# NazirNayal8/RbA

Hardware: AMD Instinct MI355X
Metric: images/sec @1024x2048 Swin-B-1dl (RbA inference hot path) (higher is better)
Workload: dtype f32 (f16x3 split-MFMA GEMMs, fp32 accumulate)

## Files before the change

### include/rba_hip.h

```cpp
#ifndef RBA_HIP_H
#define RBA_HIP_H

#include <stdint.h>

#ifdef __cplusplus
extern "C" {
#endif

int rba_hip_version(void);

int rba_set_concurrent_streams(int n);

int rba_reduce_f32(const float* mask, const float* cls_prob, float* rba, float* sem_seg, int32_t* argmax,
                   int Q, int K, int64_t HW, int score_mode, void* stream);

int rba_reduce_ws_f32(const float* mask, const float* cls_prob, float* rba, float* sem_seg, int32_t* argmax, int Q, int K,
                      int64_t HW, int score_mode, void* workspace, void* stream);

int rba_reduce_up4_f32(const float* mask_lowres, const float* cls_prob, float* rba, float* sem_seg,
                       int32_t* argmax, int Q, int K, int h, int w, int crop_h, int crop_w, int score_mode, void* stream);

int rba_resample_bilinear_f32(const float* in, const float* add, float* out, int C, int h, int w, int H, int W,
                              void* stream);

int rba_ms_deform_attn_fwd_f32(const float* value, const int64_t* spatial_shapes, const int64_t* level_start_index,
                               const float* sampling_loc, const float* attn_weight, float* out,
                               int N, int S, int M, int D, int L, int Lq, int P, void* stream);
int rba_ms_deform_attn_fwd_f64(const double* value, const int64_t* spatial_shapes, const int64_t* level_start_index,
                               const double* sampling_loc, const double* attn_weight, double* out,
                               int N, int S, int M, int D, int L, int Lq, int P, void* stream);

int rba_ms_deform_attn_bwd_f32(const float* value, const int64_t* spatial_shapes, const int64_t* level_start_index,
                               const float* sampling_loc, const float* attn_weight, const float* grad_out,
                               float* grad_value, float* grad_sampling_loc, float* grad_attn_weight,
                               int N, int S, int M, int D, int L, int Lq, int P, void* stream);
int rba_ms_deform_attn_bwd_f64(const double* value, const int64_t* spatial_shapes, const int64_t* level_start_index,
                               const double* sampling_loc, const double* attn_weight, const double* grad_out,
                               double* grad_value, double* grad_sampling_loc, double* grad_attn_weight,
                               int N, int S, int M, int D, int L, int Lq, int P, void* stream);

int rba_msda_prepare_f32(const float* raw, const float* reference_points, const int64_t* spatial_shapes, float* loc, float* attw,
                         int64_t rows, int M, int L, int P, void* stream);

int rba_msda_fused_f32(const float* value, const int64_t* spatial_shapes, const int64_t* level_start_index, const float* raw,
                       const float* reference_points, float* out, int N, int S, int M, int D, int L, int Lq, int P, void* stream);

int64_t rba_masked_xattn_workspace_bytes(int B, int Q, int S, int nH);
int rba_masked_xattn_f32(const float* q, const float* k, const float* v, const float* mask_logits, float* out,
                         float* workspace, int B, int Q, int S, int nH, int hd, void* stream);

int rba_mask_logits_f32(const float* embed, const float* feat, float* out, int B, int Q, int C, int64_t N,
                        void* stream);
int rba_mask_logits_f16x3_f32(const float* embed, const float* feat, float* out, int B, int Q, int C, int64_t N,
                              void* stream);

int rba_swin_window_attn_f32(const float* qkv, const float* qkv_bias, const float* bias, const float* bias_frag,
                             float* out, int B, int H, int W, int nH, int hd, int ws, int shift, void* stream);
int64_t rba_swin_bias_fragments_elems(int nH, int ws);
int rba_swin_bias_fragments_f32(const float* bias, float* frag, int nH, int ws, void* stream);

int64_t rba_group_norm_workspace_bytes(int B, int C, int HW, int G);
int rba_group_norm_f32(const float* x, const float* gamma, const float* beta, float* y, float* workspace,
                       int B, int C, int HW, int G, float eps, int relu, void* stream);

int64_t rba_group_norm_nhwc_workspace_bytes(int B, int P, int C, int G);
int rba_group_norm_nhwc_f32(const float* x, const float* gamma, const float* beta, float* y, float* workspace, int B, int P, int C,
                            int G, float eps, int relu, void* stream);
int rba_resample_bilinear_nhwc_f32(const float* in, const float* add, float* out, int C, int h, int w, int H, int W, void* stream);

int rba_add_layer_norm_f32(const float* x, const float* t, const float* t_bias, const float* gamma, const float* beta,
                           float* sum_out, float* y, int64_t rows, int C, float eps, void* stream);

int rba_merge_layer_norm_f32(const float* x, const float* gamma, const float* beta, float* y, int B, int H, int W, int Cin, float eps,
                             void* stream);

int rba_skinny_linear_f32(const float* x, const float* weight, const float* bias, float* out, int M, int N, int K,
                          int relu, void* stream);
int rba_skinny_linear_add_f32(const float* x, const float* x_add, int add_cols, const float* weight, const float* bias, float* out,
                              int M, int N, int K, int relu, int seg_n, void* stream);

int rba_split_weight_bf16x3(const float* weight, void* packed, int N, int K, void* stream);
int rba_split_linear_f32(const float* x, const void* weight_packed, const float* bias, float* out, int64_t M, int N, int K,
                         int act, void* stream);

int rba_split_weight_f16x2(const float* weight, void* packed, int N, int K, void* stream);
int rba_split_linear_f16x3_f32(const float* x, const void* weight_packed, const float* bias, float* out, int64_t M, int N, int K,
                               int act, void* stream);
int rba_split_linear_f16x3_res_f32(const float* x, const void* weight_packed, const float* bias, const float* residual, float* out,
                                   int64_t M, int N, int K, void* stream);

int rba_add_layer_norm_frag_f32(const float* x, const float* t, const float* t_bias, const float* gamma, const float* beta,
                                float* sum_out, void* y_frag, int64_t rows, int C, float eps, void* stream);
int rba_split_linear_f16x3_frag_f32(const void* x_frag, const void* weight_packed, const float* bias, const float* residual, float* out,
                                    int64_t M, int N, int K, int act, void* stream);
int rba_swin_window_attn_split_out_f32(const float* qkv, const float* qkv_bias, const float* bias_frag, void* out_frag, int B, int H, int W,
                                       int nH, int hd, int ws, int shift, void* stream);
int rba_swin_attn_block_supported(int C, int ws);
int64_t rba_swin_attn_block_weight_bytes(int C);
int rba_swin_attn_block_pack_f32(const float* qkv_weight, const float* proj_weight, void* image, int C, void* stream);
int rba_swin_attn_block_f32(float* x, float* y2, const float* norm1_weight, const float* norm1_bias, float eps1, const void* weight_image,
                            const float* qkv_bias, const float* bias_frag, const float* proj_bias, const float* norm2_weight,
                            const float* norm2_bias, float eps2, int B, int H, int W, int C, int ws, int shift, void* stream);
int rba_swin_attn_qkv_supported(int C, int ws);
int rba_swin_attn_qkv_split_out_f32(const float* x, void* out_frag, const float* norm1_weight, const float* norm1_bias, float eps1,
                                    const void* weight_image, const float* qkv_bias, const float* bias_frag, int B, int H, int W, int C, int ws,
                                    int shift, void* stream);
int rba_resample_bilinear_nhwc_split_out_f32(const float* in, const float* add, void* out_frag, int C, int h, int w, int H, int W,
                                             int64_t row0, void* stream);

int rba_resample_bilinear_nhwc_gn_f32(const float* in, const float* in_mr, const float* in_gamma, const float* in_beta, int in_relu,
                                      const float* add, const float* add_mr, const float* add_gamma, const float* add_beta, void* out,
                                      int split_out, int C, int G, int h, int w, int H, int W, int64_t row0, void* stream);
int rba_group_norm_nhwc_stats_f32(const float* x, float* mr, float* workspace, int B, int P, int C, int G, float eps, void* stream);
int rba_conv3x3_nhwc_f16x3_split_in_f32(const void* x_frag, const void* weight_packed, const float* bias, float* out, int B, int H, int W,
                                        int C, int N, void* stream);
int rba_swin_mlp_fused_f16x3_f32(const float* x, const void* w1_packed, const float* b1, const void* w2_packed, const float* b2,
                                 const float* residual, float* out, int64_t M, int C, int HID, void* stream);
int rba_swin_mlp_fused_ln_f16x3_f32(float* x, const float* norm_weight, const float* norm_bias, float eps, const void* w1_packed, const float* b1,
                                    const void* w2_packed, const float* b2, int64_t M, int C, int HID, void* stream);
int rba_split_linear_f16x3_gelu_split_out(const void* x, int x_is_split, const void* weight_packed, const float* bias, void* out_frag,
                                          int64_t M, int N, int K, void* stream);

int rba_split_linear_nchw_out_f32(const float* x, const void* weight_packed, const float* bias, float* out, int64_t M, int N,
                                  int K, int rows_per_image, void* stream);

int rba_split_linear_nchw_out_f16x3_f32(const float* x, const void* weight_packed, const float* bias, float* out, int64_t M, int N, int K,
                                        int rows_per_image, void* stream);

int rba_split_linear_nchw_out_gn_f16x3_f32(const float* x, const float* mr, const float* gamma, const float* beta, int G, int relu,
                                           const void* weight_packed, const float* bias, float* out, int64_t M, int N, int K,
                                           int rows_per_image, void* stream);

int rba_conv3x3_nhwc_f32(const float* x, const void* weight_packed, const float* bias, float* out, int B, int H, int W, int C,
                         int N, void* stream);

int rba_conv3x3_nhwc_f16x3_f32(const float* x, const void* weight_packed, const float* bias, float* out, int B, int H, int W, int C,
                               int N, void* stream);

int rba_split_linear_f16x3_gn_moments_f32(const float* x, const void* weight_packed, const float* bias, float* out, int64_t M, int N, int K,
                                          int rows_per_image, int G, float* moments, void* stream);
int rba_conv3x3_nhwc_f16x3_split_in_gn_moments_f32(const void* x_frag, const void* weight_packed, const float* bias, float* out, int B, int H,
                                                   int W, int C, int N, int G, float* moments, void* stream);
int rba_group_norm_nhwc_merge_f32(const float* moments, float* mr, int B, int G, int splits, float eps, void* stream);

int rba_patch_im2col_u8(const uint8_t* image, float* out, int h, int w, int Hp, int Wp, const float* mean, const float* std, void* stream);
int rba_patch_im2col_f32(const float* image, float* out, int h, int w, int Hp, int Wp, const float* mean, const float* std, void* stream);

int rba_gaussian_blur_f32(const float* in, float* out, int H, int W, int kernel_size, float sigma, void* stream);

int rba_quad_mean_f32(const float* v, float* out, int64_t rows, int S, void* stream);
int rba_softmax_drop_last_f32(const float* logits, float* prob, int64_t rows, int K1, void* stream);

int rba_threshold_u8(const float* score, uint8_t* out, int64_t n, float threshold, void* stream);
int rba_morph3x3_u8(const uint8_t* in, uint8_t* out, int H, int W, int dilate, void* stream);
int rba_ccl4_roots_i32(const uint8_t* mask, int32_t* roots, int H, int W, void* stream);

int rba_bn_relu_conv1x1_f32(const float* x, const float* scale, const float* shift, const float* weight, const float* bias, float* out,
// ... 23 lines not shown
```

### rba_amd/_lib.py

```python
import ctypes
import os

_HERE = os.path.dirname(os.path.abspath(__file__))
LIB_PATH = os.environ.get("RBA_HIP_LIB") or os.path.join(_HERE, "csrc", "librba_hip.so")
KNOBS_LIB_PATH = os.path.join(_HERE, "csrc", "librba_hip_knobs.so")

_c_f32p = ctypes.c_void_p
_i = ctypes.c_int
_i64 = ctypes.c_int64
_vp = ctypes.c_void_p

SIGNATURES = {
    "rba_hip_version": [],
    "rba_set_concurrent_streams": [_i],
    "rba_reduce_f32": [_vp, _vp, _vp, _vp, _vp, _i, _i, _i64, _i, _vp],
    "rba_reduce_ws_f32": [_vp, _vp, _vp, _vp, _vp, _i, _i, _i64, _i, _vp, _vp],
    "rba_reduce_up4_f32": [_vp, _vp, _vp, _vp, _vp, _i, _i, _i, _i, _i, _i, _i, _vp],
    "rba_resample_bilinear_f32": [_vp, _vp, _vp, _i, _i, _i, _i, _i, _vp],
    "rba_ms_deform_attn_fwd_f32": [_vp, _vp, _vp, _vp, _vp, _vp, _i, _i, _i, _i, _i, _i, _i, _vp],
    "rba_ms_deform_attn_fwd_f64": [_vp, _vp, _vp, _vp, _vp, _vp, _i, _i, _i, _i, _i, _i, _i, _vp],
    "rba_ms_deform_attn_bwd_f32": [_vp, _vp, _vp, _vp, _vp, _vp, _vp, _vp, _vp, _i, _i, _i, _i, _i, _i, _i, _vp],
    "rba_ms_deform_attn_bwd_f64": [_vp, _vp, _vp, _vp, _vp, _vp, _vp, _vp, _vp, _i, _i, _i, _i, _i, _i, _i, _vp],
    "rba_msda_prepare_f32": [_vp, _vp, _vp, _vp, _vp, _i64, _i, _i, _i, _vp],
    "rba_resample_bilinear_nhwc_gn_f32": [_vp, _vp, _vp, _vp, _i, _vp, _vp, _vp, _vp, _vp, _i, _i, _i, _i, _i, _i, _i, _i64, _vp],
    "rba_group_norm_nhwc_stats_f32": [_vp, _vp, _vp, _i, _i, _i, _i, ctypes.c_float, _vp],
    "rba_msda_fused_f32": [_vp, _vp, _vp, _vp, _vp, _vp, _i, _i, _i, _i, _i, _i, _i, _vp],
    "rba_masked_xattn_workspace_bytes": [_i, _i, _i, _i],
    "rba_masked_xattn_f32": [_vp, _vp, _vp, _vp, _vp, _vp, _i, _i, _i, _i, _i, _vp],
    "rba_mask_logits_f32": [_vp, _vp, _vp, _i, _i, _i, _i64, _vp],
    "rba_mask_logits_f16x3_f32": [_vp, _vp, _vp, _i, _i, _i, _i64, _vp],
    "rba_swin_window_attn_f32": [_vp, _vp, _vp, _vp, _vp, _i, _i, _i, _i, _i, _i, _i, _vp],
    "rba_swin_window_attn_split_out_f32": [_vp, _vp, _vp, _vp, _i, _i, _i, _i, _i, _i, _i, _vp],
    "rba_swin_bias_fragments_elems": [_i, _i],
    "rba_swin_attn_block_supported": [_i, _i],
    "rba_swin_attn_block_weight_bytes": [_i],
    "rba_swin_attn_qkv_supported": [_i, _i],
    "rba_swin_attn_qkv_split_out_f32": [_vp, _vp, _vp, _vp, ctypes.c_float, _vp, _vp, _vp, _i, _i, _i, _i, _i, _i, _vp],
    "rba_swin_attn_block_pack_f32": [_vp, _vp, _vp, _i, _vp],
    "rba_swin_attn_block_f32": [_vp, _vp, _vp, _vp, ctypes.c_float, _vp, _vp, _vp, _vp, _vp, _vp, ctypes.c_float, _i, _i, _i, _i, _i, _i, _vp],
    "rba_swin_bias_fragments_f32": [_vp, _vp, _i, _i, _vp],
    "rba_skinny_linear_f32": [_vp, _vp, _vp, _vp, _i, _i, _i, _i, _vp],
    "rba_skinny_linear_add_f32": [_vp, _vp, _i, _vp, _vp, _vp, _i, _i, _i, _i, _i, _vp],
    "rba_split_weight_bf16x3": [_vp, _vp, _i, _i, _vp],
    "rba_split_linear_f32": [_vp, _vp, _vp, _vp, _i64, _i, _i, _i, _vp],
    "rba_split_weight_f16x2": [_vp, _vp, _i, _i, _vp],
    "rba_split_linear_f16x3_f32": [_vp, _vp, _vp, _vp, _i64, _i, _i, _i, _vp],
    "rba_split_linear_f16x3_res_f32": [_vp, _vp, _vp, _vp, _vp, _i64, _i, _i, _vp],
    "rba_split_linear_f16x3_frag_f32": [_vp, _vp, _vp, _vp, _vp, _i64, _i, _i, _i, _vp],
    "rba_swin_mlp_fused_f16x3_f32": [_vp, _vp, _vp, _vp, _vp, _vp, _vp, _i64, _i, _i, _vp],
    "rba_swin_mlp_fused_ln_f16x3_f32": [_vp, _vp, _vp, ctypes.c_float, _vp, _vp, _vp, _vp, _i64, _i, _i, _vp],
    "rba_split_linear_f16x3_gelu_split_out": [_vp, _i, _vp, _vp, _vp, _i64, _i, _i, _vp],
    "rba_split_linear_nchw_out_f32": [_vp, _vp, _vp, _vp, _i64, _i, _i, _i, _vp],
    "rba_split_linear_nchw_out_f16x3_f32": [_vp, _vp, _vp, _vp, _i64, _i, _i, _i, _vp],
    "rba_split_linear_f16x3_gn_moments_f32": [_vp, _vp, _vp, _vp, _i64, _i, _i, _i, _i, _vp, _vp],
    "rba_conv3x3_nhwc_f16x3_split_in_gn_moments_f32": [_vp, _vp, _vp, _vp, _i, _i, _i, _i, _i, _i, _vp, _vp],
    "rba_group_norm_nhwc_merge_f32": [_vp, _vp, _i, _i, _i, ctypes.c_float, _vp],
    "rba_split_linear_nchw_out_gn_f16x3_f32": [_vp, _vp, _vp, _vp, _i, _i, _vp, _vp, _vp, _i64, _i, _i, _i, _vp],
    "rba_conv3x3_nhwc_f32": [_vp, _vp, _vp, _vp, _i, _i, _i, _i, _i, _vp],
    "rba_conv3x3_nhwc_f16x3_f32": [_vp, _vp, _vp, _vp, _i, _i, _i, _i, _i, _vp],
    "rba_conv3x3_nhwc_f16x3_split_in_f32": [_vp, _vp, _vp, _vp, _i, _i, _i, _i, _i, _vp],
    "rba_resample_bilinear_nhwc_split_out_f32": [_vp, _vp, _vp, _i, _i, _i, _i, _i, _i64, _vp],
    "rba_patch_im2col_u8": [_vp, _vp, _i, _i, _i, _i, _vp, _vp, _vp],
    "rba_patch_im2col_f32": [_vp, _vp, _i, _i, _i, _i, _vp, _vp, _vp],
    "rba_group_norm_nhwc_workspace_bytes": [_i, _i, _i, _i],
    "rba_group_norm_nhwc_f32": [_vp, _vp, _vp, _vp, _vp, _i, _i, _i, _i, ctypes.c_float, _i, _vp],
    "rba_resample_bilinear_nhwc_f32": [_vp, _vp, _vp, _i, _i, _i, _i, _i, _vp],
    "rba_bn_relu_conv1x1_f32": [_vp, _vp, _vp, _vp, _vp, _vp, _i, _i, _i, _i64, _vp],
    "rba_resample_bilinear_ac_f32": [_vp, _vp, _i, _i, _i, _i, _i, _vp],
    "rba_gaussian_blur_f32": [_vp, _vp, _i, _i, _i, ctypes.c_float, _vp],
    "rba_quad_mean_f32": [_vp, _vp, _i64, _i, _vp],
    "rba_softmax_drop_last_f32": [_vp, _vp, _i64, _i, _vp],
    "rba_threshold_u8": [_vp, _vp, _i64, ctypes.c_float, _vp],
    "rba_morph3x3_u8": [_vp, _vp, _i, _i, _i, _vp],
    "rba_ccl4_roots_i32": [_vp, _vp, _i, _i, _vp],
    "rba_add_layer_norm_f32": [_vp, _vp, _vp, _vp, _vp, _vp, _vp, _i64, _i, ctypes.c_float, _vp],
    "rba_add_layer_norm_frag_f32": [_vp, _vp, _vp, _vp, _vp, _vp, _vp, _i64, _i, ctypes.c_float, _vp],
    "rba_merge_layer_norm_f32": [_vp, _vp, _vp, _vp, _i, _i, _i, _i, ctypes.c_float, _vp],
    "rba_group_norm_workspace_bytes": [_i, _i, _i, _i],
    "rba_group_norm_f32": [_vp, _vp, _vp, _vp, _vp, _i, _i, _i, _i, ctypes.c_float, _i, _vp],
    "rba_token_linear_pack_f16x2": [_vp, _vp, _i, _i, _vp],
    "rba_token_linear_f32": [_vp, _vp, _vp, _vp, _vp, _vp, _vp, ctypes.c_float, _vp, _i64, _i, _i, _i, _vp],
    "rba_token_linear_multi_f32": [_vp, _vp, _i, _i64, _i, _vp],
}

class TokenLinearProblem(ctypes.Structure):
    _fields_ = [("x_add", ctypes.c_void_p), ("packed", ctypes.c_void_p), ("bias", ctypes.c_void_p), ("out", ctypes.c_void_p),
                ("N", ctypes.c_int), ("ld_out", ctypes.c_int), ("act", ctypes.c_int)]


EXPECTED_ABI = 191

_lib = None


class RbaHipError(RuntimeError):
    pass


def load():
    global _lib
    if _lib is not None:
        return _lib
    _lib = _open(LIB_PATH)
    return _lib


_handles = {}


def _open(path):
    if path in _handles:
        return _handles[path]
    import torch
    if not os.path.exists(path):
        raise RbaHipError(
            f"{path} not found: build it with `python -m rba_amd.csrc.build` (hipcc --offload-arch=gfx950; --knobs for the knobs build). "
            "rba_amd has no CPU or PyTorch fallback for its HIP kernels.")
    lib = ctypes.CDLL(path)
    for name, argtypes in SIGNATURES.items():
        try:
            fn = getattr(lib, name)
        except AttributeError as e:
            raise RbaHipError(f"{path} does not export {name}; rebuild it") from e
        fn.argtypes = argtypes
        fn.restype = ctypes.c_int64 if name.endswith(("_bytes", "_elems")) else ctypes.c_int
    abi = int(lib.rba_hip_version())
    if abi != EXPECTED_ABI:
        raise RbaHipError(f"{path} has ABI version {abi}, these bindings are written for {EXPECTED_ABI}; rebuild it "
                          "(python -m rba_amd.csrc.build)")
    _handles[path] = lib
    return lib


class use_library:

    def __init__(self, path):
        self.path = path

    def __enter__(self):
        global _lib
        self.prev = _lib
        _lib = _open(self.path)
        return _lib

    def __exit__(self, *exc):
        global _lib
        _lib = self.prev
        return False


def knob(name):
    try:
        return ctypes.c_int.in_dll(load(), name)
    except ValueError as e:
        raise RbaHipError(f"{name} is a compile-time constant in the product library: run on the knobs build (RBA_HIP_LIB={KNOBS_LIB_PATH} or "
                          "rba_amd._lib.use_library(KNOBS_LIB_PATH); python -m rba_amd.csrc.build --knobs)") from e


def hip_error_string(code: int) -> str:
    try:
# ... 12 lines not shown
```

### rba_amd/csrc/layer_norm.hip

```cpp
#include "common.h"
#include "../../include/rba_hip.h"

namespace {

struct MergeGeom {
  int H, W, Cin;
};

template <int G, int NV, bool MERGE = false, bool FRAG = false, int WAVES = 4>
__global__ __launch_bounds__(64 * WAVES) void add_layer_norm_kernel(const float* x, const float* __restrict__ t,
                                                             const float* __restrict__ tb, const float* __restrict__ gamma,
                                                             const float* __restrict__ beta, float* sum_out ,
                                                             float* __restrict__ y, int64_t rows, int C, float eps,
                                                             MergeGeom mg = MergeGeom{0, 0, 0}) {
  constexpr int RPW = 64 / G;
  const int lane = threadIdx.x & 63, sub = lane % G, rsel = lane / G;
  const int64_t row = ((int64_t)blockIdx.x * WAVES + (threadIdx.x >> 6)) * RPW + rsel;
  constexpr bool TR = FRAG && WAVES == 8 && G == 64;
  __shared__ __attribute__((aligned(16))) rba_u32x4 tr_lds[TR ? NV * 64 * 8 : 1];
  const bool rvalid = row < rows;
  const int64_t base = (rvalid ? row : 0) * C;
  const int nv4 = C >> 2;
  int mi = 0, mj = 0;
  int64_t mb = 0;
// ... 49 lines not shown
    }
  }
#pragma unroll
  for (int o = G / 2; o > 0; o >>= 1) sq += __shfl_xor(sq, o, RBA_WAVE);
  const float rstd = 1.0f / sqrtf(sq / (float)C + eps);
  if (!TR && !rvalid) return;
#pragma unroll
  for (int j = 0; j < NV; ++j) {
    const int c4 = sub + j * G;
    if (c4 < nv4) {
      if (sum_out && rvalid) *reinterpret_cast<f32x4*>(sum_out + base + 4 * c4) = v[j];
      const f32x4 gj = EARLY ? g4[EARLY ? j : 0] : *reinterpret_cast<const f32x4*>(gamma + 4 * c4);
      const f32x4 bj = EARLY ? b4[EARLY ? j : 0] : *reinterpret_cast<const f32x4*>(beta + 4 * c4);
      const f32x4 o = (v[j] - mean) * rstd * gj + bj;
      if (FRAG) {
        uint32_t h[2], l[2];
        rba_split_f16x2(o.x, o.y, h[0], l[0]);
        rba_split_f16x2(o.z, o.w, h[1], l[1]);
        const bool odd = c4 & 1;
        const uint32_t s0 = odd ? h[0] : l[0], s1 = odd ? h[1] : l[1];
        const uint32_t r0 = __builtin_amdgcn_mov_dpp(s0, 0xB1, 0xf, 0xf, true), r1 = __builtin_amdgcn_mov_dpp(s1, 0xB1, 0xf, 0xf, true);
        const rba_u32x4 piece = odd ? (rba_u32x4){r0, r1, l[0], l[1]} : (rba_u32x4){h[0], h[1], r0, r1};
        const int k8 = c4 >> 1;
        if (TR) {
          const int pcol = (((k8 >> 2) * 4 + (k8 & 1) * 2 + (odd ? 1 : 0)) << 1) + ((k8 >> 1) & 1);
          const int r8 = threadIdx.x >> 6;
          tr_lds[pcol * 8 + (r8 ^ (pcol & 7))] = piece;
        } else {
          const int64_t off = ((row >> 5) * (int64_t)(C >> 5) + (k8 >> 2)) * 4096 + ((k8 & 1) * 2 + (odd ? 1 : 0)) * 1024 +
                              (((k8 >> 1) & 1) * 32 + (int)(row & 31)) * 16;
          *reinterpret_cast<rba_u32x4*>(reinterpret_cast<char*>(y) + off) = piece;
        }
      } else {
        *reinterpret_cast<f32x4*>(y + base + 4 * c4) = o;
      }
    }
  }
  if (TR) {
    __syncthreads();
    const int64_t row0 = (int64_t)blockIdx.x * 8;
    char* img = reinterpret_cast<char*>(y) + ((row0 >> 5) * (int64_t)(C >> 5)) * 4096 + (int)(row0 & 31) * 16;
    const int npc = nv4;
    for (int u = threadIdx.x; u < npc * 8; u += 64 * WAVES) {
      const int pcol = u >> 3, r8 = u & 7;
      const int x = pcol >> 1;
      if (row0 + r8 < rows)
        *reinterpret_cast<rba_u32x4*>(img + (int64_t)(x >> 2) * 4096 + (x & 3) * 1024 + (pcol & 1) * 512 + r8 * 16) = tr_lds[pcol * 8 + (r8 ^ (pcol & 7))];
    }
  }
}

template <int G, int NV, bool FRAG = false>
int launch(const float* x, const float* t, const float* tb, const float* gamma, const float* beta, float* sum_out, float* y,
           int64_t rows, int C, float eps, hipStream_t st) {
  const int64_t rpb = 4 * (64 / G);
  const int64_t blocks = (rows + rpb - 1) / rpb;
  if (blocks > 0x7fffffffLL) return (int)hipErrorInvalidValue;
  hipLaunchKernelGGL((add_layer_norm_kernel<G, NV, false, FRAG>), dim3((unsigned)blocks), dim3(256), 0, st, x, t, tb, gamma, beta, sum_out, y,
                     rows, C, eps);
  return rba_launch_status();
}

template <int NV>
int launch_frag8(const float* x, const float* t, const float* tb, const float* gamma, const float* beta, float* sum_out, float* y,
                 int64_t rows, int C, float eps, hipStream_t st) {
  const int64_t blocks = (rows + 7) / 8;
  if (blocks > 0x7fffffffLL) return (int)hipErrorInvalidValue;
  hipLaunchKernelGGL((add_layer_norm_kernel<64, NV, false, true, 8>), dim3((unsigned)blocks), dim3(512), 0, st, x, t, tb, gamma, beta, sum_out,
                     y, rows, C, eps);
  return rba_launch_status();
}

template <int G, int NV>
int launch_merge(const float* x, const float* gamma, const float* beta, float* y, int64_t rows, int C, float eps, MergeGeom mg,
                 hipStream_t st) {
  const int64_t rpb = 4 * (64 / G);
  const int64_t blocks = (rows + rpb - 1) / rpb;
  if (blocks > 0x7fffffffLL) return (int)hipErrorInvalidValue;
  hipLaunchKernelGGL((add_layer_norm_kernel<G, NV, true>), dim3((unsigned)blocks), dim3(256), 0, st, x, nullptr, nullptr, gamma, beta, nullptr,
                     y, rows, C, eps, mg);
  return rba_launch_status();
}

}

extern "C" int rba_merge_layer_norm_f32(const float* x, const float* gamma, const float* beta, float* y, int B, int H, int W, int Cin,
                                        float eps, void* stream) {
  RBA_CHECK_ARG(B >= 0 && H >= 1 && W >= 1 && Cin >= 4 && Cin % 4 == 0 && 4 * Cin <= 8192);
  if (B == 0) return 0;
  RBA_CHECK_ARG(x && gamma && beta && y);
  RBA_CHECK_ARG((((uintptr_t)x | (uintptr_t)gamma | (uintptr_t)beta | (uintptr_t)y) & 15) == 0);
  rba_begin();
  hipStream_t st = (hipStream_t)stream;
  const int C = 4 * Cin, nv4 = C / 4;
  const int64_t rows = (int64_t)B * ((H + 1) / 2) * ((W + 1) / 2);
  const MergeGeom mg{H, W, Cin};
#define RBA_L(G, NV) return launch_merge<G, NV>(x, gamma, beta, y, rows, C, eps, mg, st)
  if (nv4 <= 16) RBA_L(16, 1);
  if (nv4 <= 32) RBA_L(32, 1);
  if (nv4 <= 64) RBA_L(64, 1);
  if (nv4 <= 128) RBA_L(64, 2);
  if (nv4 <= 256) RBA_L(64, 4);
  if (nv4 <= 512) RBA_L(64, 8);
  if (nv4 <= 1024) RBA_L(64, 16);
  RBA_L(64, 32);
#undef RBA_L
}

extern "C" int rba_add_layer_norm_f32(const float* x, const float* t, const float* t_bias, const float* gamma, const float* beta,
                                      float* sum_out, float* y, int64_t rows, int C, float eps, void* stream) {
  RBA_CHECK_ARG(rows >= 0 && C >= 4 && C % 4 == 0 && C <= 8192);
  if (rows == 0) return 0;
  RBA_CHECK_ARG(x && gamma && beta && y);
  RBA_CHECK_ARG((((uintptr_t)x | (uintptr_t)t | (uintptr_t)t_bias | (uintptr_t)gamma | (uintptr_t)beta | (uintptr_t)sum_out |
                  (uintptr_t)y) & 15) == 0);
  rba_begin();
  hipStream_t st = (hipStream_t)stream;
  const int nv4 = C / 4;
#define RBA_L(G, NV) return launch<G, NV>(x, t, t_bias, gamma, beta, sum_out, y, rows, C, eps, st)
  if (nv4 <= 16) RBA_L(16, 1);
  if (nv4 <= 32) RBA_L(32, 1);
  if (nv4 <= 64) RBA_L(64, 1);
  if (nv4 <= 128) RBA_L(64, 2);
  if (nv4 <= 256) RBA_L(64, 4);
  if (nv4 <= 512) RBA_L(64, 8);
  if (nv4 <= 1024) RBA_L(64, 16);
  RBA_L(64, 32);
#undef RBA_L
}

extern "C" int rba_add_layer_norm_frag_f32(const float* x, const float* t, const float* t_bias, const float* gamma, const float* beta,
                                           float* sum_out, void* y_frag, int64_t rows, int C, float eps, void* stream) {
  RBA_CHECK_ARG(rows >= 0 && C >= 32 && C % 32 == 0 && C <= 8192);
  if (rows == 0) return 0;
  RBA_CHECK_ARG(x && gamma && beta && y_frag);
  RBA_CHECK_ARG((((uintptr_t)x | (uintptr_t)t | (uintptr_t)t_bias | (uintptr_t)gamma | (uintptr_t)beta | (uintptr_t)sum_out |
                  (uintptr_t)y_frag) & 15) == 0);
  rba_begin();
  hipStream_t st = (hipStream_t)stream;
  const int nv4 = C / 4;
  float* y = reinterpret_cast<float*>(y_frag);
  if (nv4 > 64 && nv4 <= 128) return launch_frag8<2>(x, t, t_bias, gamma, beta, sum_out, y, rows, C, eps, st);
  if (nv4 > 128 && nv4 <= 256) return launch_frag8<4>(x, t, t_bias, gamma, beta, sum_out, y, rows, C, eps, st);
  if (nv4 > 256 && nv4 <= 512) return launch_frag8<8>(x, t, t_bias, gamma, beta, sum_out, y, rows, C, eps, st);
#define RBA_L(G, NV) return launch<G, NV, true>(x, t, t_bias, gamma, beta, sum_out, y, rows, C, eps, st)
  if (nv4 <= 16) RBA_L(16, 1);
  if (nv4 <= 32) RBA_L(32, 1);
  if (nv4 <= 64) RBA_L(64, 1);
  if (nv4 <= 128) RBA_L(64, 2);
  if (nv4 <= 256) RBA_L(64, 4);
  if (nv4 <= 512) RBA_L(64, 8);
  if (nv4 <= 1024) RBA_L(64, 16);
  RBA_L(64, 32);
#undef RBA_L
}
```

### rba_amd/modeling/backbone/swin.py

```python
from types import SimpleNamespace

import torch
import torch.nn as nn
import torch.nn.functional as F

from ... import ops
from ...lru import derived
from ...registry import BACKBONE_REGISTRY


def relative_position_index(ws: int) -> torch.Tensor:
    ar = torch.arange(ws)
    gy, gx = torch.meshgrid(ar, ar, indexing="ij")
    gy, gx = gy.reshape(-1), gx.reshape(-1)
    dy = gy[:, None] - gy[None, :] + (ws - 1)
    dx = gx[:, None] - gx[None, :] + (ws - 1)
    return dy * (2 * ws - 1) + dx


class WindowAttention(nn.Module):
    def __init__(self, dim, window_size, num_heads):
        super().__init__()
        self.dim, self.window_size, self.num_heads = dim, window_size, num_heads
        self.relative_position_bias_table = nn.Parameter(torch.zeros((2 * window_size - 1) ** 2, num_heads))
# ... 101 lines not shown
    def __init__(self, dim, depth, num_heads, window_size, mlp_ratio, downsample):
        super().__init__()
        self.blocks = nn.ModuleList(
            SwinTransformerBlock(dim, num_heads, window_size, 0 if i % 2 == 0 else window_size // 2, mlp_ratio)
            for i in range(depth))
        self.downsample = PatchMerging(dim) if downsample else None


class PatchEmbed(nn.Module):
    def __init__(self, patch_size, in_chans, embed_dim):
        super().__init__()
        self.patch_size = patch_size
        self.proj = nn.Conv2d(in_chans, embed_dim, kernel_size=patch_size, stride=patch_size)
        self.norm = nn.LayerNorm(embed_dim)

    def forward(self, x):
        ps = self.patch_size
        _, _, H, W = x.shape
        if W % ps or H % ps:
            x = F.pad(x, (0, (ps - W % ps) % ps, 0, (ps - H % ps) % ps))
        B, Cin, H, W = x.shape
        Wh, Ww = H // ps, W // ps
        cols = x.reshape(B, Cin, Wh, ps, Ww, ps).permute(0, 2, 4, 1, 3, 5).reshape(B, Wh * Ww, Cin * ps * ps).contiguous()
        x = ops.linear(cols, self._linear_view())
        return ops.add_layer_norm(x, self.norm.weight, self.norm.bias, self.norm.eps)[1], Wh, Ww

    def _linear_view(self):
        w, b = self.proj.weight, self.proj.bias
        return derived(self, "linear_view", (w, b), lambda: SimpleNamespace(weight=w.detach().reshape(w.shape[0], -1), bias=b))

    def fused_ok(self):
        w = self.proj.weight
        return self.patch_size == 4 and w.shape[1] == 3 and w.is_cuda and w.dtype == torch.float32 and ops.SPLIT_MODE == "f16x3"

    def forward_images(self, images, mean, std, Hp, Wp):
        w = self.proj.weight

        def build():
            w64 = torch.zeros((w.shape[0], 64), dtype=torch.float32, device=w.device)
            w64[:, :48] = w.detach().reshape(w.shape[0], 48)
            return ops.split_weight(w64, mode="f16x3")

        planes = derived(self, "planes64", (w,), build)
        cols = torch.stack([ops.patch_im2col(im, mean, std, Hp, Wp) for im in images]) if len(images) > 1 \
            else ops.patch_im2col(images[0], mean, std, Hp, Wp)[None]
        x = ops.split_linear(cols, planes, self.proj.bias, out_features=w.shape[0])
        return ops.add_layer_norm(x, self.norm.weight, self.norm.bias, self.norm.eps)[1], Hp // 4, Wp // 4


@BACKBONE_REGISTRY.register()
class D2SwinTransformer(nn.Module):

    def __init__(self, arch):
        super().__init__()
        E, depths = arch["embed_dim"], arch["depths"]
        self.patch_embed = PatchEmbed(arch["patch_size"], 3, E)
        self.layers = nn.ModuleList(
            BasicLayer(E * 2 ** i, depths[i], arch["num_heads"][i], arch["window_size"], arch["mlp_ratio"],
                       downsample=i < len(depths) - 1) for i in range(len(depths)))
        self.num_features = [E * 2 ** i for i in range(len(depths))]
        for i, c in enumerate(self.num_features):
            self.add_module(f"norm{i}", nn.LayerNorm(c))

    @property
    def size_divisibility(self):
        return 32

    def forward_images(self, images, mean, std, Hp, Wp):
        return self._stages(*self.patch_embed.forward_images(images, mean, std, Hp, Wp))

    def forward(self, x):
        if x.dim() != 4:
            raise ValueError(f"SwinTransformer takes an input of shape (N, C, H, W). Got {tuple(x.shape)} instead!")
        return self._stages(*self.patch_embed(x))

    def _stages(self, x, Wh, Ww):
        outs = {}
        for i, layer in enumerate(self.layers):
            pending = None
            for blk in layer.blocks:
                x, pending = blk(x, Wh, Ww, pending)
            norm = getattr(self, f"norm{i}")
            t, tb = pending if pending is not None else (None, None)
            x, y = ops.add_layer_norm(x, norm.weight, norm.bias, norm.eps, t, tb, inplace_sum=True)
            outs[f"res{i + 2}"] = y.view(-1, Wh, Ww, self.num_features[i]).permute(0, 3, 1, 2)
            if layer.downsample is not None:
                x = layer.downsample(x, Wh, Ww)
                Wh, Ww = (Wh + 1) // 2, (Ww + 1) // 2
        return outs
```

### rba_amd/ops.py

```python
import contextlib
import ctypes
import threading
import functools
import math
import os

import torch

from . import _lib
from ._lib import RbaHipError
from .lru import derived


def _stream():
    return torch.cuda.current_stream().cuda_stream


def _cuda_tensors(args):
    for a in args:
        if isinstance(a, torch.Tensor):
            if a.is_cuda:
                yield a
        elif isinstance(a, (list, tuple)):
            yield from _cuda_tensors(a)
# ... 378 lines not shown
    _chk(x, "x")
    _chk(weight, "weight", dim=1)
    _chk(bias, "bias", dim=1)
    C = x.shape[-1]
    if weight.numel() != C or bias.numel() != C:
        raise RbaHipError("weight / bias must match the last dimension")
    rows = x.numel() // C if C else 0
    if residual is not None:
        _chk(residual, "residual")
        if tuple(residual.shape) != tuple(x.shape):
            raise RbaHipError("residual must have x's shape")
    if residual_bias is not None:
        _chk(residual_bias, "residual_bias", dim=1)
        if residual_bias.numel() != C:
            raise RbaHipError("residual_bias must have C elements")
    has_sum = residual is not None or residual_bias is not None
    s = x if (not has_sum or inplace_sum) else torch.empty_like(x)
    if frag:
        if C % 32:
            raise RbaHipError("add_layer_norm(frag=True) needs C % 32 == 0")
        y = SplitActivations.empty(tuple(x.shape), x.device)
        _lib.check(lib.rba_add_layer_norm_frag_f32(_p(x), _p(residual), _p(residual_bias), _p(weight), _p(bias),
                                                   _p(s) if has_sum else 0, _p(y.data), rows, C, float(eps), _stream()),
                   "rba_add_layer_norm_frag_f32")
        return s, y
    y = torch.empty_like(x)
    _lib.check(lib.rba_add_layer_norm_f32(_p(x), _p(residual), _p(residual_bias), _p(weight), _p(bias),
                                          _p(s) if has_sum else 0, _p(y), rows, C, float(eps), _stream()),
               "rba_add_layer_norm_f32")
    return s, y


@_hip_op
def msda_prepare(raw, reference_points, spatial_shapes, M, L, P):
    lib = _lib.load()
    _chk(raw, "raw", dim=3)
    _chk(reference_points, "reference_points", dim=4)
    _chk(spatial_shapes, "spatial_shapes", torch.int64, 2)
    N, Lq, W3 = raw.shape
    if W3 != 3 * M * L * P or tuple(reference_points.shape) != (N, Lq, L, 2) or spatial_shapes.shape[0] != L:
        raise RbaHipError("msda_prepare: shapes do not match")
    loc = torch.empty((N, Lq, M, L, P, 2), dtype=torch.float32, device=raw.device)
    attw = torch.empty((N, Lq, M, L, P), dtype=torch.float32, device=raw.device)
    _lib.check(lib.rba_msda_prepare_f32(_p(raw), _p(reference_points), _p(spatial_shapes), _p(loc), _p(attw), N * Lq, M, L, P, _stream()),
               "rba_msda_prepare_f32")
    return loc, attw


def msda_fused_ok(D, L, P, S=None, M=None):
    return D == 32 and P == 4 and L in (1, 3) and (S is None or M is None or S * M * 128 < (1 << 32))


@_hip_op
def msda_fused(value, spatial_shapes, level_start_index, raw, reference_points, M, L, P):
    lib = _lib.load()
    _chk(value, "value", dim=4)
    _chk(spatial_shapes, "spatial_shapes", torch.int64, 2)
    _chk(level_start_index, "level_start_index", torch.int64, 1)
    _chk(raw, "raw", dim=3)
    _chk(reference_points, "reference_points", dim=4)
    N, S, M2, D = value.shape
    _, Lq, W3 = raw.shape
    if (M2 != M or not msda_fused_ok(D, L, P, S, M) or W3 != 3 * M * L * P or raw.shape[0] != N or tuple(reference_points.shape) != (N, Lq, L, 2)
            or spatial_shapes.shape[0] != L or level_start_index.shape[0] != L):
        raise RbaHipError("msda_fused: shapes do not match (head_dim 32, P = 4, L in {1, 3})")
    out = torch.empty((N, Lq, M * D), dtype=torch.float32, device=value.device)
    _lib.check(lib.rba_msda_fused_f32(_p(value), _p(spatial_shapes), _p(level_start_index), _p(raw), _p(reference_points), _p(out),
                                      N, S, M, D, L, Lq, P, _stream()), "rba_msda_fused_f32")
    return out


@_hip_op
def merge_layer_norm(x, H, W, weight, bias, eps=1e-5):
    lib = _lib.load()
    _chk(x, "x", dim=3)
    _chk(weight, "weight", dim=1)
    _chk(bias, "bias", dim=1)
    B, L, C = x.shape
    if L != H * W or C % 4 or weight.numel() != 4 * C or bias.numel() != 4 * C:
        raise RbaHipError("merge_layer_norm needs x [B, H*W, C] (C % 4 == 0) and a LayerNorm over 4C channels")
    y = torch.empty((B, ((H + 1) // 2) * ((W + 1) // 2), 4 * C), dtype=torch.float32, device=x.device)
    _lib.check(lib.rba_merge_layer_norm_f32(_p(x), _p(weight), _p(bias), _p(y), B, H, W, C, float(eps), _stream()), "rba_merge_layer_norm_f32")
    return y


@_hip_op
def skinny_linear(x, weight, bias=None, relu=False, x_add=None, add_cols=None, segments=1, out=None):
    lib = _lib.load()
    _chk(x, "x")
    _chk(weight, "weight", dim=2)
    K = x.shape[-1]
    N = weight.shape[0]
    M = x.numel() // K if K else 0
    if weight.shape[1] != K or K % 32 or M > 128:
        raise RbaHipError("skinny_linear needs weight [N,K], K % 32 == 0 and at most 128 rows")
    if bias is not None:
        _chk(bias, "bias", dim=1)
        if bias.numel() != N:
            raise RbaHipError("bias must have N elements")
    segments = int(segments)
    if segments < 1 or N % segments:
        raise RbaHipError("segments must divide N")
    if out is not None:
        _chk(out, "out")
        if segments != 1 or tuple(out.shape) != tuple(x.shape[:-1]) + (N,):
            raise RbaHipError("out must be a contiguous fp32 [..., N] tensor with x's leading shape (segments = 1)")
    if x_add is None and segments == 1:
        if out is None:
            out = torch.empty(tuple(x.shape[:-1]) + (N,), dtype=torch.float32, device=x.device)
        _lib.check(lib.rba_skinny_linear_f32(_p(x), _p(weight), _p(bias), _p(out), M, N, K, int(bool(relu)), _stream()),
                   "rba_skinny_linear_f32")
        return out
    if x_add is not None:
        _chk(x_add, "x_add")
        if tuple(x_add.shape) != tuple(x.shape):
            raise RbaHipError("x_add must have x's shape")
    add_cols = N if add_cols is None else int(add_cols)
    if add_cols % 16 or not 0 <= add_cols <= N:
        raise RbaHipError("add_cols must be a multiple of 16 in [0, N]")
    seg_n = N // segments
    if out is not None:
        _lib.check(lib.rba_skinny_linear_add_f32(_p(x), _p(x_add), add_cols, _p(weight), _p(bias), _p(out), M, N, K, int(bool(relu)), 0, _stream()),
                   "rba_skinny_linear_add_f32")
        return out
    out = torch.empty((segments,) + tuple(x.shape[:-1]) + (seg_n,), dtype=torch.float32, device=x.device)
    _lib.check(lib.rba_skinny_linear_add_f32(_p(x), _p(x_add), add_cols, _p(weight), _p(bias), _p(out), M, N, K, int(bool(relu)),
                                             seg_n if segments > 1 else 0, _stream()), "rba_skinny_linear_add_f32")
    return out[0] if segments == 1 else tuple(out[i] for i in range(segments))


class SplitActivations:
    __slots__ = ("data", "shape")

    def __init__(self, data, shape):
        self.data, self.shape = data, tuple(shape)

    @staticmethod
    def empty(shape, device):
        K = shape[-1]
        M = 1
        for d in shape[:-1]:
            M *= d
        return SplitActivations(torch.empty((((M + 31) // 32) * 32 * K,), dtype=torch.int32, device=device), shape)

    @property
    def device(self):
        return self.data.device

    def numel(self):
        n = 1
        for d in self.shape:
            n *= d
        return n

    @staticmethod
    def pack(x):
        K = x.shape[-1]
        x2 = x.reshape(-1, K).float()
        M = x2.shape[0]
        Mp = (M + 31) // 32 * 32
        xp = torch.zeros((Mp, K), dtype=torch.float32, device=x.device)
        xp[:M] = x2
        h = xp.half()
        l = ((xp - h.float()) * 2048.0).half()
        hl = torch.stack([h, l], 0).reshape(2, Mp // 32, 32, K // 32, 2, 2, 8)
        img = hl.permute(1, 3, 5, 0, 4, 2, 6).contiguous()
# ... 728 lines not shown
```

Measured before the change: 147.9.

## Fuse stage-end add+LayerNorm with patch-merge gather and LayerNorm

Adds a stage-boundary kernel that adds the pending residual, applies the stage output LayerNorm, gathers 2x2 tokens into LDS, and applies the patch-merging LayerNorm in one pass. Where possible it writes the merged result directly in the split f16 fragment layout consumed by the reduction GEMM. This removes the intermediate summed-tensor write, its re-read by the merge kernel, and a separate split/pack step. In exchange the residual sum x is no longer written back, and the kernel carries extra LDS use and template variants.

Measured after the change: 149.1 (median of 6 runs). About the same (+0.8%).

```diff
diff --git a/include/rba_hip.h b/include/rba_hip.h
--- a/include/rba_hip.h
+++ b/include/rba_hip.h
@@ -73,6 +73,10 @@
 
 int rba_merge_layer_norm_f32(const float* x, const float* gamma, const float* beta, float* y, int B, int H, int W, int Cin, float eps,
                              void* stream);
+
+int rba_stage_boundary_f32(const float* x, const float* t, const float* t_bias, const float* gamma_c, const float* beta_c, float eps_c,
+                           float* y_stage, const float* gamma_m, const float* beta_m, float eps_m, void* y_merge, int frag, int B, int H,
+                           int W, int Cin, void* stream);
 
 int rba_skinny_linear_f32(const float* x, const float* weight, const float* bias, float* out, int M, int N, int K,
                           int relu, void* stream);
diff --git a/rba_amd/_lib.py b/rba_amd/_lib.py
--- a/rba_amd/_lib.py
+++ b/rba_amd/_lib.py
@@ -76,6 +76,7 @@
     "rba_add_layer_norm_f32": [_vp, _vp, _vp, _vp, _vp, _vp, _vp, _i64, _i, ctypes.c_float, _vp],
     "rba_add_layer_norm_frag_f32": [_vp, _vp, _vp, _vp, _vp, _vp, _vp, _i64, _i, ctypes.c_float, _vp],
     "rba_merge_layer_norm_f32": [_vp, _vp, _vp, _vp, _i, _i, _i, _i, ctypes.c_float, _vp],
+    "rba_stage_boundary_f32": [_vp, _vp, _vp, _vp, _vp, ctypes.c_float, _vp, _vp, _vp, ctypes.c_float, _vp, _i, _i, _i, _i, _i, _vp],
     "rba_group_norm_workspace_bytes": [_i, _i, _i, _i],
     "rba_group_norm_f32": [_vp, _vp, _vp, _vp, _vp, _i, _i, _i, _i, ctypes.c_float, _i, _vp],
     "rba_token_linear_pack_f16x2": [_vp, _vp, _i, _i, _vp],
diff --git a/rba_amd/csrc/layer_norm.hip b/rba_amd/csrc/layer_norm.hip
--- a/rba_amd/csrc/layer_norm.hip
+++ b/rba_amd/csrc/layer_norm.hip
@@ -155,6 +155,181 @@
   return rba_launch_status();
 }
 
+__device__ __forceinline__ float sb_rounded(float p) {
+  asm("" : "+v"(p));
+  return p;
+}
+
+template <bool FUSED>
+__device__ __forceinline__ float sb_sq4(f32x4 d) {
+  if (FUSED) return __builtin_fmaf(d.x, d.x, sb_rounded(d.y * d.y)) + __builtin_fmaf(d.z, d.z, sb_rounded(d.w * d.w));
+  return (sb_rounded(d.x * d.x) + sb_rounded(d.y * d.y)) + (sb_rounded(d.z * d.z) + sb_rounded(d.w * d.w));
+}
+
+template <int G, int NV>
+__device__ __forceinline__ void sb_row_stats(const f32x4 (&v)[NV], float sum, int sub, int nv4, int C, float eps, float& mean, float& rstd) {
+#pragma unroll
+  for (int o = G / 2; o > 0; o >>= 1) sum += __shfl_xor(sum, o, RBA_WAVE);
+  mean = sum / (float)C;
+  float sq = 0.f;
+#pragma unroll
+  for (int j = 0; j < NV; ++j)
+    if (sub + j * G < nv4) sq += sb_sq4<NV == 1>(v[j] - mean);
+#pragma unroll
+  for (int o = G / 2; o > 0; o >>= 1) sq += __shfl_xor(sq, o, RBA_WAVE);
+  rstd = 1.0f / sqrtf(sq / (float)C + eps);
+}
+
+__device__ __forceinline__ f32x4 sb_apply(f32x4 v, float mean, float rstd, f32x4 g, f32x4 b) {
+  const f32x4 u = (v - mean) * rstd;
+  return (f32x4){__builtin_fmaf(u.x, g.x, b.x), __builtin_fmaf(u.y, g.y, b.y), __builtin_fmaf(u.z, g.z, b.z), __builtin_fmaf(u.w, g.w, b.w)};
+}
+
+__device__ __forceinline__ float sb_lane_sum(f32x4 a) { return (a.x + a.y) + (a.z + a.w); }
+
+__device__ __forceinline__ void sb_store_frag(f32x4 o, int c4, rba_u32x4* tr_lds) {
+  uint32_t h[2], l[2];
+  rba_split_f16x2(o.x, o.y, h[0], l[0]);
+  rba_split_f16x2(o.z, o.w, h[1], l[1]);
+  const bool odd = c4 & 1;
+  const uint32_t s0 = odd ? h[0] : l[0], s1 = odd ? h[1] : l[1];
+  const uint32_t r0 = __builtin_amdgcn_mov_dpp(s0, 0xB1, 0xf, 0xf, true), r1 = __builtin_amdgcn_mov_dpp(s1, 0xB1, 0xf, 0xf, true);
+  const rba_u32x4 piece = odd ? (rba_u32x4){r0, r1, l[0], l[1]} : (rba_u32x4){h[0], h[1], r0, r1};
+  const int k8 = c4 >> 1;
+  const int pcol = (((k8 >> 2) * 4 + (k8 & 1) * 2 + (odd ? 1 : 0)) << 1) + ((k8 >> 1) & 1);
+  const int r8 = threadIdx.x >> 6;
+  tr_lds[pcol * 8 + (r8 ^ (pcol & 7))] = piece;
+}
+
+__device__ __forceinline__ void sb_flush_frag(const rba_u32x4* tr_lds, float* y, int64_t row0, int64_t rows, int C, int nthreads) {
+  char* img = reinterpret_cast<char*>(y) + ((row0 >> 5) * (int64_t)(C >> 5)) * 4096 + (int)(row0 & 31) * 16;
+  const int npc = C >> 2;
+  for (int u = threadIdx.x; u < npc * 8; u += nthreads) {
+    const int pcol = u >> 3, r8 = u & 7;
+    const int x = pcol >> 1;
+    if (row0 + r8 < rows)
+      *reinterpret_cast<rba_u32x4*>(img + (int64_t)(x >> 2) * 4096 + (x & 3) * 1024 + (pcol & 1) * 512 + r8 * 16) = tr_lds[pcol * 8 + (r8 ^ (pcol & 7))];
+  }
+}
+
+template <int GC, int NVC, int GM, int NVM, bool FRAG, int WAVES>
+__global__ __launch_bounds__(64 * WAVES) void stage_boundary_kernel(const float* __restrict__ x, const float* __restrict__ t,
+                                                             const float* __restrict__ tb, const float* __restrict__ gamma_c,
+                                                             const float* __restrict__ beta_c, float* __restrict__ yc,
+                                                             const float* __restrict__ gamma_m, const float* __restrict__ beta_m,
+                                                             float* __restrict__ ym, int64_t rows , float eps_c, float eps_m,
+                                                             MergeGeom mg) {
+  static_assert(!FRAG || (GM == 64 && WAVES == 8), "the split image is written through the transposed stores");
+  constexpr int RPWM = 64 / GM, RPWC = 64 / GC, PASSES = 4 * RPWM / RPWC;
+  static_assert(PASSES >= 1 && PASSES * RPWC == 4 * RPWM, "a wave's source tokens fill whole passes");
+  extern __shared__ __attribute__((aligned(16))) float park[];
+  const int lane = threadIdx.x & 63, wave = threadIdx.x >> 6;
+  const int Cin = mg.Cin, C = 4 * Cin;
+  const int H2 = (mg.H + 1) >> 1, W2 = (mg.W + 1) >> 1;
+  const int64_t mrow0 = ((int64_t)blockIdx.x * WAVES + wave) * RPWM;
+  {
+    const int sub = lane % GC, rsel = lane / GC, nv4 = Cin >> 2;
+#pragma unroll
+    for (int p = 0; p < PASSES; ++p) {
+      const int slot = p * RPWC + rsel, rm = slot >> 2, seg = slot & 3;
+      const int64_t mrow = mrow0 + rm;
+      bool valid = mrow < rows;
+      const int64_t r = valid ? mrow : 0;
+      const int64_t bimg = r / ((int64_t)H2 * W2);
+      const int rem = (int)(r - bimg * H2 * W2);
+      const int mi = rem / W2, mj = rem - mi * W2;
+      const int si = 2 * mi + (seg & 1), sj = 2 * mj + (seg >> 1);
+      valid = valid && si < mg.H && sj < mg.W;
+      const int64_t base = valid ? ((bimg * mg.H + si) * mg.W + sj) * Cin : 0;
+      f32x4 v[NVC];
+      float sum = 0.f;
+#pragma unroll
+      for (int j = 0; j < NVC; ++j) {
+        const int c4 = sub + j * GC;
+        f32x4 a = {0.f, 0.f, 0.f, 0.f};
+        if (c4 < nv4 && valid) {
+          a = *reinterpret_cast<const f32x4*>(x + base + 4 * c4);
+          if (t) a += *reinterpret_cast<const f32x4*>(t + base + 4 * c4);
+          if (tb) a += *reinterpret_cast<const f32x4*>(tb + 4 * c4);
+          sum += sb_lane_sum(a);
+        }
+        v[j] = a;
+      }
+      float mean, rstd;
+      sb_row_stats<GC, NVC>(v, sum, sub, nv4, Cin, eps_c, mean, rstd);
+      float* prow = park + (int64_t)(wave * RPWM + rm) * C + seg * Cin;
+#pragma unroll
+      for (int j = 0; j < NVC; ++j) {
+        const int c4 = sub + j * GC;
+        if (c4 < nv4) {
+          *reinterpret_cast<f32x4*>(prow + 4 * c4) = v[j];
+          if (yc && valid)
+            *reinterpret_cast<f32x4*>(yc + base + 4 * c4) = sb_apply(v[j], mean, rstd, *reinterpret_cast<const f32x4*>(gamma_c + 4 * c4),
+                                                                     *reinterpret_cast<const f32x4*>(beta_c + 4 * c4));
+        }
+      }
+    }
+  }
+  __syncthreads();
+  const int sub = lane % GM, rsel = lane / GM, nv4 = C >> 2;
+  const int64_t row = mrow0 + rsel;
+  const bool rvalid = row < rows;
+  f32x4 v[NVM];
+  float sum = 0.f;
+#pragma unroll
+  for (int j = 0; j < NVM; ++j) {
+    const int c4 = sub + j * GM;
+    f32x4 a = {0.f, 0.f, 0.f, 0.f};
+    if (c4 < nv4) {
+      a = *reinterpret_cast<const f32x4*>(park + (int64_t)(wave * RPWM + rsel) * C + 4 * c4);
+      sum += sb_lane_sum(a);
+    }
+    v[j] = a;
+  }
+  float mean, rstd;
+  sb_row_stats<GM, NVM>(v, sum, sub, nv4, C, eps_m, mean, rstd);
+  rba_u32x4* tr_lds = reinterpret_cast<rba_u32x4*>(park);
+  if (FRAG) __syncthreads();
+#pragma unroll
+  for (int j = 0; j < NVM; ++j) {
+    const int c4 = sub + j * GM;
+    if (c4 < nv4) {
+      const f32x4 o = sb_apply(v[j], mean, rstd, *reinterpret_cast<const f32x4*>(gamma_m + 4 * c4), *reinterpret_cast<const f32x4*>(beta_m + 4 * c4));
+      if (FRAG) {
+        sb_store_frag(o, c4, tr_lds);
+      } else if (rvalid) {
+        *reinterpret_cast<f32x4*>(ym + row * C + 4 * c4) = o;
+      }
+    }
+  }
+  if (FRAG) {
+    __syncthreads();
+    sb_flush_frag(tr_lds, ym, (int64_t)blockIdx.x * 8, rows, C, 64 * WAVES);
+  }
+}
+
+template <int GC, int NVC, int GM, int NVM>
+int launch_boundary(const float* x, const float* t, const float* tb, const float* gamma_c, const float* beta_c, float* yc, const float* gamma_m,
+                    const float* beta_m, float* ym, int frag, int64_t rows, float eps_c, float eps_m, MergeGeom mg, hipStream_t st) {
+  const int C = 4 * mg.Cin;
+  if constexpr (GM == 64 && NVM >= 2 && NVM <= 8) {
+    if (frag) {
+      const int64_t blocks = (rows + 7) / 8;
+      if (blocks > 0x7fffffffLL) return (int)hipErrorInvalidValue;
+      hipLaunchKernelGGL((stage_boundary_kernel<GC, NVC, GM, NVM, true, 8>), dim3((unsigned)blocks), dim3(512), (size_t)NVM * 64 * 8 * 16, st, x, t,
+                         tb, gamma_c, beta_c, yc, gamma_m, beta_m, ym, rows, eps_c, eps_m, mg);
+      return rba_launch_status();
+    }
+  }
+  if (frag) return (int)hipErrorInvalidValue;
+  const int64_t rpb = 4 * (64 / GM);
+  const int64_t blocks = (rows + rpb - 1) / rpb;
+  if (blocks > 0x7fffffffLL) return (int)hipErrorInvalidValue;
+  hipLaunchKernelGGL((stage_boundary_kernel<GC, NVC, GM, NVM, false, 4>), dim3((unsigned)blocks), dim3(256), (size_t)rpb * C * sizeof(float), st, x,
+                     t, tb, gamma_c, beta_c, yc, gamma_m, beta_m, ym, rows, eps_c, eps_m, mg);
+  return rba_launch_status();
+}
+
 }
 
 extern "C" int rba_merge_layer_norm_f32(const float* x, const float* gamma, const float* beta, float* y, int B, int H, int W, int Cin,
@@ -227,3 +402,30 @@
   RBA_L(64, 32);
 #undef RBA_L
 }
+
+extern "C" int rba_stage_boundary_f32(const float* x, const float* t, const float* t_bias, const float* gamma_c, const float* beta_c, float eps_c,
+                                      float* y_stage, const float* gamma_m, const float* beta_m, float eps_m, void* y_merge, int frag, int B, int H,
+                                      int W, int Cin, void* stream) {
+  RBA_CHECK_ARG(B >= 0 && H >= 1 && W >= 1 && Cin >= 4 && Cin % 4 == 0 && Cin <= 1024);
+  RBA_CHECK_ARG(!frag || (Cin > 64 && Cin <= 512 && Cin % 8 == 0));
+  if (B == 0) return 0;
+  RBA_CHECK_ARG(x && gamma_c && beta_c && gamma_m && beta_m && y_merge);
+  RBA_CHECK_ARG((((uintptr_t)x | (uintptr_t)t | (uintptr_t)t_bias | (uintptr_t)gamma_c | (uintptr_t)beta_c | (uintptr_t)y_stage |
+                  (uintptr_t)gamma_m | (uintptr_t)beta_m | (uintptr_t)y_merge) & 15) == 0);
+  rba_begin();
+  hipStream_t st = (hipStream_t)stream;
+  const int nv4 = Cin / 4;
+  const int64_t rows = (int64_t)B * ((H + 1) / 2) * ((W + 1) / 2);
+  const MergeGeom mg{H, W, Cin};
+#define RBA_L(GC, NVC, GM, NVM) \
+  return launch_boundary<GC, NVC, GM, NVM>(x, t, t_bias, gamma_c, beta_c, y_stage, gamma_m, beta_m, reinterpret_cast<float*>(y_merge), frag, rows, \
+                                           eps_c, eps_m, mg, st)
+  if (nv4 <= 4) RBA_L(16, 1, 16, 1);
+  if (nv4 <= 8) RBA_L(16, 1, 32, 1);
+  if (nv4 <= 16) RBA_L(16, 1, 64, 1);
+  if (nv4 <= 32) RBA_L(32, 1, 64, 2);
+  if (nv4 <= 64) RBA_L(64, 1, 64, 4);
+  if (nv4 <= 128) RBA_L(64, 2, 64, 8);
+  RBA_L(64, 4, 64, 16);
+#undef RBA_L
+}
diff --git a/rba_amd/modeling/backbone/swin.py b/rba_amd/modeling/backbone/swin.py
--- a/rba_amd/modeling/backbone/swin.py
+++ b/rba_amd/modeling/backbone/swin.py
@@ -207,9 +207,16 @@
                 x, pending = blk(x, Wh, Ww, pending)
             norm = getattr(self, f"norm{i}")
             t, tb = pending if pending is not None else (None, None)
-            x, y = ops.add_layer_norm(x, norm.weight, norm.bias, norm.eps, t, tb, inplace_sum=True)
+            C, merged = self.num_features[i], None
+            if layer.downsample is not None and x.is_cuda and x.dim() == 3 and ops.stage_boundary_ok(C):
+                pm = layer.downsample
+                M2 = x.shape[0] * ((Wh + 1) // 2) * ((Ww + 1) // 2)
+                y, merged = ops.stage_boundary(x, Wh, Ww, (norm.weight, norm.bias, norm.eps), (pm.norm.weight, pm.norm.bias, pm.norm.eps), t, tb,
+                                               frag=ops.stage_boundary_takes_frag(C) and ops.linear_takes_split(M2, 2 * C, 4 * C))
+            else:
+                x, y = ops.add_layer_norm(x, norm.weight, norm.bias, norm.eps, t, tb, inplace_sum=True)
             outs[f"res{i + 2}"] = y.view(-1, Wh, Ww, self.num_features[i]).permute(0, 3, 1, 2)
             if layer.downsample is not None:
-                x = layer.downsample(x, Wh, Ww)
+                x = ops.linear(merged, layer.downsample.reduction) if merged is not None else layer.downsample(x, Wh, Ww)
                 Wh, Ww = (Wh + 1) // 2, (Ww + 1) // 2
         return outs
diff --git a/rba_amd/ops.py b/rba_amd/ops.py
--- a/rba_amd/ops.py
+++ b/rba_amd/ops.py
@@ -484,6 +484,47 @@
     y = torch.empty((B, ((H + 1) // 2) * ((W + 1) // 2), 4 * C), dtype=torch.float32, device=x.device)
     _lib.check(lib.rba_merge_layer_norm_f32(_p(x), _p(weight), _p(bias), _p(y), B, H, W, C, float(eps), _stream()), "rba_merge_layer_norm_f32")
     return y
+
+
+STAGE_BOUNDARY_FUSED = os.environ.get("RBA_STAGE_BOUNDARY_FUSED", "1") != "0"
+
+
+def stage_boundary_ok(C):
+    return STAGE_BOUNDARY_FUSED and C % 4 == 0 and 4 <= C <= 1024
+
+
+def stage_boundary_takes_frag(C):
+    return C % 8 == 0 and 64 < C <= 512
+
+
+@_hip_op
+def stage_boundary(x, H, W, norm, merge_norm, residual=None, residual_bias=None, want_stage_out=True, frag=False):
+    lib = _lib.load()
+    _chk(x, "x", dim=3)
+    B, L, C = x.shape
+    (gc, bc, eps_c), (gm, bm, eps_m) = norm, merge_norm
+    for t_, n_, k_ in ((gc, "norm.weight", C), (bc, "norm.bias", C), (gm, "merge_norm.weight", 4 * C), (bm, "merge_norm.bias", 4 * C)):
+        _chk(t_, n_, dim=1)
+        if t_.numel() != k_:
+            raise RbaHipError(f"{n_} must have {k_} elements")
+    if L != H * W or C % 4 or not 4 <= C <= 1024:
+        raise RbaHipError("stage_boundary needs x [B, H*W, C] with C % 4 == 0 and C <= 1024")
+    if residual is not None:
+        _chk(residual, "residual")
+        if tuple(residual.shape) != tuple(x.shape):
+            raise RbaHipError("residual must have x's shape")
+    if residual_bias is not None:
+        _chk(residual_bias, "residual_bias", dim=1)
+        if residual_bias.numel() != C:
+            raise RbaHipError("residual_bias must have C elements")
+    if frag and not stage_boundary_takes_frag(C):
+        raise RbaHipError("stage_boundary(frag=True) needs C % 8 == 0 and 64 < C <= 512")
+    y = torch.empty_like(x) if want_stage_out else None
+    mshape = (B, ((H + 1) // 2) * ((W + 1) // 2), 4 * C)
+    m = SplitActivations.empty(mshape, x.device) if frag else torch.empty(mshape, dtype=torch.float32, device=x.device)
+    _lib.check(lib.rba_stage_boundary_f32(_p(x), _p(residual), _p(residual_bias), _p(gc), _p(bc), float(eps_c), _p(y), _p(gm), _p(bm), float(eps_m),
+                                          _p(m.data) if frag else _p(m), int(bool(frag)), B, H, W, C, _stream()), "rba_stage_boundary_f32")
+    return y, m
 
 
 @_hip_op
```
